# sisl/Crux.jl

Hardware: AMD Instinct MI355X
Metric: env-steps/sec + grad-steps/sec, PPO 2048x32 rollout (higher is better)
Workload: dtype f32

## Files before the change

### crux.jl_amd/csrc/env.hip

```cpp
#include "rollout.h"
#include "per_tree.h"

void crux_buffer_ring_advance(crux_buffer* b, int64_t N);
int32_t crux_buffer_per_on_push(crux_buffer* b, const int64_t* d_I, int64_t N);
int32_t crux_buffer_ring_ids_device(crux_buffer* b, int64_t N, int64_t* d_out);
bool crux_per_push_fused(crux_buffer* b, int64_t n, int64_t* d_ids);
bool crux_per_push_plan(crux_buffer* b, int64_t n, int* touch);
void crux_per_push_done(crux_buffer* b, int touch);

template <int IN, int OUT, int ACT, int KIND>
__global__ __launch_bounds__(64) void k_rollout_h64(RolloutArgs a_single, const RolloutArgs* __restrict__ multi) {
  __shared__ __attribute__((aligned(16))) float sh[64];
  const RolloutArgs a = multi ? multi[blockIdx.x / a_single.E] : a_single;
  const int e = multi ? (int)(blockIdx.x % a_single.E) : (int)blockIdx.x, lane = threadIdx.x;
  const NetDesc& nd = a.nd;
  constexpr int SD = KIND == CRUX_ENV_CARTPOLE ? 4 : ((KIND == CRUX_ENV_SYNTH || KIND == CRUX_ENV_SYNTH_DISCRETE) ? IN : 2);
  float w1[IN], w2[64], w3[OUT], b3[OUT];
#pragma unroll
  for (int k = 0; k < IN; ++k) w1[k] = a.p[nd.woff[0] + lane + 64 * k];
#pragma unroll
  for (int k = 0; k < 64; ++k) w2[k] = a.p[nd.woff[1] + lane + 64 * k];
#pragma unroll
  for (int o = 0; o < OUT; ++o) { w3[o] = a.p[nd.woff[2] + o + OUT * lane]; b3[o] = a.p[nd.boff[2] + o]; }
  const float b1 = a.p[nd.boff[0] + lane], b2 = a.p[nd.boff[1] + lane];
  double st[ENV_MAXSD]; float x[IN], nx[ENV_MAXOBS];
#pragma unroll
  for (int i = 0; i < SD; ++i) st[i] = a.state[(size_t)e * SD + i];
  int64_t ep_len = a.ep_len[e], n_resets = a.n_resets[e], steps_taken = a.steps_taken[e]; double sum_r = 0.0; int64_t nee = 0;
#pragma unroll
  for (int k = 0; k < IN; ++k) x[k] = a.svec[(size_t)e * IN + k];
  for (int64_t t = 0; t < a.T; ++t) {
    const int64_t j = (a.base + (int64_t)e * a.T + t) % a.C;
    if (lane == 0) {
#pragma unroll
      for (int k = 0; k < IN; ++k) a.S[(size_t)j * IN + k] = x[k];
    }
    float z[OUT];
    h64_forward<IN, OUT, ACT>(w1, w2, w3, b3, b1, b2, x, sh, lane, z);
    rollout_tail(a, z, IN, OUT, OUT, KIND, e, t, j, lane == 0, st, ep_len, n_resets, steps_taken, sum_r, nee, nx, lane);
#pragma unroll
    for (int k = 0; k < IN; ++k) x[k] = nx[k];
  }
  if (lane == 0) {
#pragma unroll
    for (int i = 0; i < SD; ++i) a.state[(size_t)e * SD + i] = st[i];
    a.ep_len[e] = ep_len; a.n_resets[e] = n_resets; a.steps_taken[e] = steps_taken;
    a.acc[2 * e] = sum_r; a.acc[2 * e + 1] = (double)nee;
#pragma unroll
    for (int k = 0; k < IN; ++k) a.svec[(size_t)e * IN + k] = x[k];
  }
}

__global__ __launch_bounds__(64) void k_rollout(RolloutArgs a) {
  __shared__ float hbuf[2][1024];
  __shared__ float sh_misc[ENV_MAXOBS + 8];
  rollout_generic_wave(a, blockIdx.x, threadIdx.x, hbuf, sh_misc);
}
__global__ __launch_bounds__(256) void k_rollout_wide(RolloutArgs a) {
  __shared__ float hbuf[2][1024];
  __shared__ float sh_misc[ENV_MAXOBS + 8];
  rollout_generic_wave<256>(a, blockIdx.x, threadIdx.x, hbuf, sh_misc);
}
__global__ __launch_bounds__(64) void k_rollout_sigma(RolloutArgs a) {
  __shared__ float hbuf[2][1024];
  __shared__ float sh_misc[ENV_MAXOBS + 8];
  rollout_generic_wave<64, true>(a, blockIdx.x, threadIdx.x, hbuf, sh_misc);
}
__global__ __launch_bounds__(256) void k_rollout_wide_sigma(RolloutArgs a) {
  __shared__ float hbuf[2][1024];
  __shared__ float sh_misc[ENV_MAXOBS + 8];
  rollout_generic_wave<256, true>(a, blockIdx.x, threadIdx.x, hbuf, sh_misc);
}

__device__ __forceinline__ void env_lds_barrier() { asm volatile("s_waitcnt lgkmcnt(0)\n\ts_barrier" ::: "memory"); }
__device__ __forceinline__ float env_readlane(const float v, const int l) { return __builtin_bit_cast(float, __builtin_amdgcn_readlane(__builtin_bit_cast(int, v), l)); }
template <int L0>
__device__ __forceinline__ void env_rl_fma8(float& acc, const float hreg, const float w0, const float w1, const float w2, const float w3, const float w4, const float w5,
                                            const float w6, const float w7) {
  int t0, t1;
  asm volatile("v_readlane_b32 %[t0], %[h], %[l0]\n\tv_readlane_b32 %[t1], %[h], %[l1]\n\t"
               "v_fmac_f32_e32 %[acc], %[t0], %[w0]\n\tv_readlane_b32 %[t0], %[h], %[l2]\n\t"
               "v_fmac_f32_e32 %[acc], %[t1], %[w1]\n\tv_readlane_b32 %[t1], %[h], %[l3]\n\t"
               "v_fmac_f32_e32 %[acc], %[t0], %[w2]\n\tv_readlane_b32 %[t0], %[h], %[l4]\n\t"
// ... 159 lines not shown
__global__ void k_env_init(int kind, int E, int od, int sd, uint64_t seed, const float* mu, const float* sigma, double* state, int64_t* ep_len,
                           int64_t* n_resets, float* svec, int fresh) {
  const int e = blockIdx.x * blockDim.x + threadIdx.x;
  if (e >= E) return;
  const int64_t nr = fresh ? 0 : n_resets[e];
  if (env_is_synth(kind)) {
    for (int i = 0; i < sd; ++i) { const crux_u32x4 x = crux_philox(seed, 16 * (uint64_t)nr + (uint64_t)(i >> 1), (uint32_t)e, CRUX_RNG_RESET);
      const double ui = (i & 1) ? crux_u32x2_to_f64(x.v[2], x.v[3]) : crux_u32x2_to_f64(x.v[0], x.v[1]); const double xi = __dadd_rn(-0.05, __dmul_rn(0.1, ui));
      state[(size_t)e * sd + i] = xi; svec[(size_t)e * od + i] = __fdiv_rn(__fsub_rn((float)xi, mu[i]), sigma[i]); }
    n_resets[e] = nr + 1; ep_len[e] = 0; return;
  }
  double st[4]; float o[4];
  st[0] = st[1] = st[2] = st[3] = 0.0; o[0] = o[1] = o[2] = o[3] = 0.f;
  env_draw_initial(kind, seed, (uint64_t)nr, (uint32_t)e, st);
#pragma unroll
  for (int i = 0; i < 4; ++i) if (i < sd) state[(size_t)e * sd + i] = st[i];
  n_resets[e] = nr + 1; ep_len[e] = 0;
  env_obs(kind, st, o);
#pragma unroll
  for (int q = 0; q < 4; ++q) if (q < od) svec[(size_t)e * od + q] = __fdiv_rn(__fsub_rn(o[q], mu[q]), sigma[q]);
}

__global__ void k_env_step(int kind, int64_t n, const double* state, const void* action, const double* uniforms, double* next_state, float* obs, float* r, uint8_t* done) {
  const int64_t j = (int64_t)blockIdx.x * blockDim.x + threadIdx.x;
  if (j >= n) return;
  if (kind == CRUX_ENV_GRIDWORLD) {
    const uint8_t* a = (const uint8_t*)action + 4 * j; int act = 0; for (int q = 0; q < 4; ++q) if (a[q]) act = q;
    double s[2] = {state[2 * j], state[2 * j + 1]}, sn[2]; float rr; uint8_t dd;
    gridworld_step(s, act, uniforms ? uniforms[j] : 0.0, sn, &rr, &dd);
    next_state[2 * j] = sn[0]; next_state[2 * j + 1] = sn[1]; obs[2 * j] = (float)sn[0]; obs[2 * j + 1] = (float)sn[1]; r[j] = rr; done[j] = dd; return;
  }
  if (kind == CRUX_ENV_CARTPOLE) {
    const uint8_t* a = (const uint8_t*)action + 2 * j; double s[4], sn[4]; for (int i = 0; i < 4; ++i) s[i] = state[4 * j + i];
    float rr; uint8_t dd; cartpole_step(s, a[1] ? 1 : 0, sn, &rr, &dd);
    for (int i = 0; i < 4; ++i) { next_state[4 * j + i] = sn[i]; obs[4 * j + i] = (float)sn[i]; } r[j] = rr; done[j] = dd;
  } else {
    double s[2] = {state[2 * j], state[2 * j + 1]}, sn[2]; float rr; uint8_t dd; float o[3];
    pendulum_step(s, ((const float*)action)[j], sn, &rr, &dd); env_obs(kind, sn, o);
    next_state[2 * j] = sn[0]; next_state[2 * j + 1] = sn[1]; obs[3 * j] = o[0]; obs[3 * j + 1] = o[1]; obs[3 * j + 2] = o[2]; r[j] = rr; done[j] = dd;
  }
}

static void env_dims(int kind, int so, int sa, int* obs, int* act, int* sd) {
  switch (kind) {
    case CRUX_ENV_CARTPOLE: *obs = 4; *act = 2; *sd = 4; break;
    case CRUX_ENV_PENDULUM: *obs = 3; *act = 1; *sd = 2; break;
    case CRUX_ENV_GRIDWORLD: *obs = 2; *act = 4; *sd = 2; break;
    case CRUX_ENV_SYNTH: case CRUX_ENV_SYNTH_DISCRETE: *obs = so; *act = sa; *sd = so; break;
    default: *obs = so; *act = sa; *sd = 1; break;
  }
}

static bool launch_rollout_h64(const NetDesc& pn, int kind, dim3 grid, hipStream_t stream, const RolloutArgs& a, const RolloutArgs* d_multi) {
#define RO_CASE(I, O, A_, K) if (pn.dims[0] == I && pn.dims[3] == O && pn.acts[0] == A_ && kind == K) { hipLaunchKernelGGL((k_rollout_h64<I, O, A_, K>), grid, dim3(64), 0, stream, a, d_multi); return true; }
  H64_SHAPES(RO_CASE)
#undef RO_CASE
  return false;
}

extern "C" {

int32_t crux_env_create(crux_ctx* ctx, int32_t kind, int32_t n_envs, int32_t max_steps, float gamma, const float* obs_mu, const float* obs_sigma,
                        uint64_t seed, int32_t synth_obs_dim, int32_t synth_act_dim, crux_env** out) {
  if (!ctx || !out) return CRUX_EINVAL;
  if (kind < CRUX_ENV_CARTPOLE || kind > CRUX_ENV_SYNTH_DISCRETE) return crux_fail(ctx, CRUX_EUNSUP, "env kind %d has no device dynamics", kind);
  if ((kind == CRUX_ENV_SYNTH || kind == CRUX_ENV_SYNTH_DISCRETE) && (synth_obs_dim < 1 || synth_obs_dim > ENV_MAXOBS || synth_act_dim < 1 || synth_act_dim > ENV_MAXOBS))
    return crux_fail(ctx, CRUX_EINVAL, "synthetic env: obs/act dims (%d, %d) must be in 1..%d", synth_obs_dim, synth_act_dim, ENV_MAXOBS);
  if (n_envs < 1 || max_steps < 1) return crux_fail(ctx, CRUX_EINVAL, "env_create: n_envs=%d max_steps=%d", n_envs, max_steps);
  crux_env* e = new crux_env(); e->ctx = ctx; e->kind = kind; e->n_envs = n_envs; e->max_steps = max_steps; e->gamma = gamma; e->seed = seed;
  env_dims(kind, synth_obs_dim, synth_act_dim, &e->obs_dim, &e->act_dim, &e->state_dim);
  const int od = e->obs_dim;
  if (hipMalloc(&e->mu, 4 * od) != hipSuccess || hipMalloc(&e->sigma, 4 * od) != hipSuccess || hipMalloc(&e->state, 8 * (size_t)n_envs * e->state_dim) != hipSuccess ||
      hipMalloc(&e->ep_len, 8 * (size_t)n_envs) != hipSuccess || hipMalloc(&e->n_resets, 8 * (size_t)n_envs) != hipSuccess ||
      hipMalloc(&e->steps_taken, 8 * (size_t)n_envs) != hipSuccess || hipMalloc(&e->svec, 4 * (size_t)n_envs * od) != hipSuccess ||
      hipMalloc(&e->acc, 16 * (size_t)n_envs) != hipSuccess) { crux_env_destroy(e); return crux_fail(ctx, CRUX_ENOMEM, "env_create: hipMalloc"); }
  std::vector<float> mu(od, 0.f), sg(od, 1.f);
  if (obs_mu) for (int i = 0; i < od; ++i) mu[i] = obs_mu[i];
  if (obs_sigma) for (int i = 0; i < od; ++i) sg[i] = obs_sigma[i];
  HIPCHK(ctx, hipMemcpyAsync(e->mu, mu.data(), 4 * od, hipMemcpyHostToDevice, ctx->stream));
  HIPCHK(ctx, hipMemcpyAsync(e->sigma, sg.data(), 4 * od, hipMemcpyHostToDevice, ctx->stream));
  HIPCHK(ctx, hipMemsetAsync(e->steps_taken, 0, 8 * (size_t)n_envs, ctx->stream));
  HIPCHK(ctx, hipMemsetAsync(e->acc, 0, 16 * (size_t)n_envs, ctx->stream));
  hipLaunchKernelGGL(k_env_init, dim3((n_envs + 63) / 64), dim3(64), 0, ctx->stream, kind, n_envs, od, e->state_dim, seed, e->mu, e->sigma, e->state, e->ep_len, e->n_resets, e->svec, 1);
  HIPCHK(ctx, hipStreamSynchronize(ctx->stream));
  *out = e; return crux_launch_check(ctx, "k_env_init");
}

int32_t crux_env_destroy(crux_env* e) {
  if (!e) return CRUX_OK;
  crux_sync_before_free(e->ctx);
  (void)hipFree(e->mu); (void)hipFree(e->sigma); (void)hipFree(e->state); (void)hipFree(e->ep_len); (void)hipFree(e->n_resets);
  (void)hipFree(e->steps_taken); (void)hipFree(e->svec); (void)hipFree(e->acc);
  delete e; return CRUX_OK;
}
int32_t crux_env_obs_dim(const crux_env* e) { return e ? e->obs_dim : -1; }
int32_t crux_env_act_dim(const crux_env* e) { return e ? e->act_dim : -1; }
int32_t crux_env_state_dim(const crux_env* e) { return e ? e->state_dim : -1; }

int32_t crux_env_reset(crux_env* e) {
  if (!e) return CRUX_EINVAL;
  hipLaunchKernelGGL(k_env_init, dim3((e->n_envs + 63) / 64), dim3(64), 0, e->ctx->stream, e->kind, e->n_envs, e->obs_dim, e->state_dim, e->seed, e->mu, e->sigma,
                     e->state, e->ep_len, e->n_resets, e->svec, 0);
  return crux_launch_check(e->ctx, "k_env_init");
}

int32_t crux_env_get_state(crux_env* e, double* state, int64_t* ep_len, int64_t* n_resets) {
  if (!e) return CRUX_EINVAL;
// ... 188 lines not shown
```

### crux.jl_amd/csrc/rollout.h

```cpp
#pragma once
#include "common.h"
#define ENV_MAXSD 32
#define ENV_MAXOBS 32
#define PI_D 3.14159265358979323846

__device__ __forceinline__ void cartpole_step(const double* s, int action, double* sn, float* r, uint8_t* done) {
  const double gravity = 9.8, masscart = 1.0, masspole = 0.1, total_mass = masspole + masscart, length = 0.5,
               polemass_length = masspole * length, force_mag = 10.0, tau = 0.02;
  double x = s[0], x_dot = s[1], theta = s[2], theta_dot = s[3];
  const double force = action == 1 ? force_mag : -force_mag;
  const double costheta = cos(theta), sintheta = sin(theta);
  const double temp = __ddiv_rn(__dadd_rn(force, __dmul_rn(__dmul_rn(polemass_length, __dmul_rn(theta_dot, theta_dot)), sintheta)), total_mass);
  const double den = __dmul_rn(length, __dsub_rn(4.0 / 3.0, __ddiv_rn(__dmul_rn(masspole, __dmul_rn(costheta, costheta)), total_mass)));
  const double thetaacc = __ddiv_rn(__dsub_rn(__dmul_rn(gravity, sintheta), __dmul_rn(costheta, temp)), den);
  const double xacc = __dsub_rn(temp, __ddiv_rn(__dmul_rn(__dmul_rn(polemass_length, thetaacc), costheta), total_mass));
  x = __dadd_rn(x, __dmul_rn(tau, x_dot)); x_dot = __dadd_rn(x_dot, __dmul_rn(tau, xacc));
  theta = __dadd_rn(theta, __dmul_rn(tau, theta_dot)); theta_dot = __dadd_rn(theta_dot, __dmul_rn(tau, thetaacc));
  sn[0] = x; sn[1] = x_dot; sn[2] = theta; sn[3] = theta_dot;
  const double xth = 2.4, thth = 12.0 * 2.0 * PI_D / 360.0;
  *done = (x < -xth || x > xth || theta < -thth || theta > thth) ? 1 : 0;
  *r = 1.0f;
}
__device__ __forceinline__ double angle_normalize(double x) { double t = fmod(x + PI_D, 2.0 * PI_D); if (t < 0) t += 2.0 * PI_D; return t - PI_D; }
__device__ __forceinline__ void pendulum_step(const double* s, float a, double* sn, float* r, uint8_t* done) {
// ... 190 lines not shown
                                             const int64_t t, const int64_t j, const bool writer, double* st, int64_t& ep_len, int64_t& n_resets,
                                             int64_t& steps_taken, double& sum_r, int64_t& nee, float* next_obs, const int par_lane = -1,
                                             const float* mu_cached = nullptr, const float* sigma_cached = nullptr) {
  const float* mu = mu_cached ? mu_cached : a.mu; const float* sg = sigma_cached ? sigma_cached : a.sigma;
  const int sd = kind == CRUX_ENV_CARTPOLE ? 4 : (env_is_synth(kind) ? od : 2);
      const uint64_t gi = a.cfg.i0 + (uint64_t)t * (uint64_t)a.E + (uint64_t)e;
      const uint64_t ctr = (uint64_t)steps_taken;
      float logprob; int ai; float aout[ENV_MAXOBS];
      if constexpr (SIGMA) rollout_head_sigma(a, z, ad, e, ctr, aout, ai, logprob); else
      rollout_head(a, z, ad, nout, e, gi, ctr, aout, ai, logprob);
      double sn[ENV_MAXSD]; float r; uint8_t done; float o[ENV_MAXOBS], spv[ENV_MAXOBS];
      if (kind == CRUX_ENV_CARTPOLE) cartpole_step(st, ai, sn, &r, &done);
      else if (kind == CRUX_ENV_PENDULUM) pendulum_step(st, aout[0], sn, &r, &done);
      else if (env_is_synth(kind)) synth_step(od, ad, kind == CRUX_ENV_SYNTH_DISCRETE, st, ai, aout, sn, &r, &done, par_lane);
      else { const crux_u32x4 xd = crux_philox(a.seed, ctr, (uint32_t)e, CRUX_RNG_ENVDYN); gridworld_step(st, ai, crux_u32x2_to_f64(xd.v[0], xd.v[1]), sn, &r, &done); }
      env_obs(kind, sn, o, od);
      for (int q = 0; q < od; ++q) spv[q] = __fdiv_rn(__fsub_rn(o[q], mu[q]), sg[q]);
      if (writer) {
        if (a.act_kind == CRUX_ACTION_DISCRETE) { uint8_t* A = (uint8_t*)a.A + (size_t)j * ad; for (int q = 0; q < ad; ++q) A[q] = aout[q] != 0.f; }
        else { float* A = (float*)a.A + (size_t)j * ad; for (int q = 0; q < ad; ++q) A[q] = aout[q]; }
        for (int q = 0; q < od; ++q) a.SP[(size_t)j * od + q] = spv[q];
        a.R[j] = r; a.D[j] = done;
        if (a.LP) a.LP[j] = logprob;
        if (a.TT) a.TT[j] = ep_len + 1;
        if (a.II) a.II[j] = (int64_t)gi + 1;
        if (a.W) a.W[j] = 1.0f;
        if (a.RET) a.RET[j] = 0.f;
        if (a.ADV) a.ADV[j] = 0.f;
        if (a.COST) a.COST[j] = env_cost(kind, od, sn);
        if (a.CADV) a.CADV[j] = 0.f;
        if (a.CRET) a.CRET[j] = 0.f;
      }
      sum_r += (double)r; steps_taken += 1;
      ep_len += 1;
      uint8_t ee = 0;
      if (done || ep_len >= a.max_steps) {
        ee = 1; ++nee;
        env_draw_initial(kind, a.seed, (uint64_t)n_resets, (uint32_t)e, st, sd); n_resets += 1; ep_len = 0;
        env_obs(kind, st, o, od);
        for (int q = 0; q < od; ++q) next_obs[q] = __fdiv_rn(__fsub_rn(o[q], mu[q]), sg[q]);
      } else {
        for (int i = 0; i < sd; ++i) st[i] = sn[i];
        for (int q = 0; q < od; ++q) next_obs[q] = spv[q];
      }
      if (a.cfg.reset_at_end && t == a.T - 1 && ep_len > 0) {
        ee = 1; ++nee;
        env_draw_initial(kind, a.seed, (uint64_t)n_resets, (uint32_t)e, st, sd); n_resets += 1; ep_len = 0;
        env_obs(kind, st, o, od);
        for (int q = 0; q < od; ++q) next_obs[q] = __fdiv_rn(__fsub_rn(o[q], mu[q]), sg[q]);
      }
      if (writer) a.EE[j] = ee;
}

template <int CTRL> __device__ __forceinline__ float env_dpp(float v) {
  return __builtin_bit_cast(float, __builtin_amdgcn_update_dpp(0, __builtin_bit_cast(int, v), CTRL, 0xf, 0xf, true));
}
__device__ __forceinline__ float env_wave_sum_uniform(float v) {
  v += env_dpp<0x128>(v); v += env_dpp<0x124>(v); v += env_dpp<0x122>(v); v += env_dpp<0x121>(v);
  float a0 = v, b0 = v;
  asm volatile("s_nop 1\n\tv_permlane16_swap_b32 %0, %1\n\ts_nop 1" : "+v"(a0), "+v"(b0));
  a0 = a0 + b0; b0 = a0;
  asm volatile("s_nop 1\n\tv_permlane32_swap_b32 %0, %1\n\ts_nop 1" : "+v"(a0), "+v"(b0));
  return __builtin_bit_cast(float, __builtin_amdgcn_readfirstlane(__builtin_bit_cast(int, a0 + b0)));
}
template <int IN, int OUT, int ACT>
__device__ __forceinline__ void h64_forward(const float (&w1)[IN], const float (&w2)[64], const float (&w3)[OUT], const float (&b3)[OUT], const float b1, const float b2,
                                            const float (&x)[IN], float* sh, const int lane, float (&z)[OUT]) {
    float acc = 0.f;
#pragma unroll
    for (int k = 0; k < IN; ++k) acc = fmaf(w1[k], x[k], acc);
    sh[lane] = crux_act(ACT, acc + b1);
    __builtin_amdgcn_fence(__ATOMIC_ACQ_REL, "wavefront"); __builtin_amdgcn_wave_barrier();
    acc = 0.f;
#pragma unroll
    for (int k4 = 0; k4 < 16; ++k4) { const float4 hv = *(const float4*)&sh[4 * k4];
      acc = fmaf(w2[4 * k4], hv.x, acc); acc = fmaf(w2[4 * k4 + 1], hv.y, acc); acc = fmaf(w2[4 * k4 + 2], hv.z, acc); acc = fmaf(w2[4 * k4 + 3], hv.w, acc); }
    __builtin_amdgcn_fence(__ATOMIC_ACQ_REL, "wavefront"); __builtin_amdgcn_wave_barrier();
    const float h2 = crux_act(ACT, acc + b2);
#pragma unroll
    for (int o = 0; o < OUT; ++o) z[o] = env_wave_sum_uniform(w3[o] * h2) + b3[o];
}
#define RO_WAVE_SYNC() do { __builtin_amdgcn_fence(__ATOMIC_ACQ_REL, "wavefront"); __builtin_amdgcn_wave_barrier(); } while (0)
template <int NT>
__device__ __forceinline__ int rollout_generic_forward(const RolloutArgs& a, const int lane, float (*hbuf)[1024]) {
    const NetDesc& nd = a.nd;
    int cur = 0;
    for (int l = 0; l < nd.L; ++l) {
      const int in = nd.dims[l], out = nd.dims[l + 1], act = nd.acts[l];
      const float* Wl = a.p + nd.woff[l]; const float* bl = a.p + nd.boff[l];
      for (int o = lane; o < out; o += NT) {
        float accv = 0.f; int k = 0;
        if (NT > 64) {
          for (; k + 32 <= in; k += 32) {
            float wv[32];
#pragma unroll
            for (int u = 0; u < 32; ++u) wv[u] = Wl[o + out * (k + u)];
#pragma unroll
            for (int u = 0; u < 32; ++u) accv = fmaf(wv[u], hbuf[cur][k + u], accv); } }
        for (; k + 8 <= in; k += 8) {
          float wv[8];
#pragma unroll
          for (int u = 0; u < 8; ++u) wv[u] = Wl[o + out * (k + u)];
#pragma unroll
          for (int u = 0; u < 8; ++u) accv = fmaf(wv[u], hbuf[cur][k + u], accv); }
        for (; k < in; ++k) accv = fmaf(Wl[o + out * k], hbuf[cur][k], accv);
        hbuf[cur ^ 1][o] = crux_act(act, accv + bl[o]);
// ... 69 lines not shown
```

### crux.jl_amd/csrc/switches.h

```cpp
#pragma once
#include <cstdlib>
struct CruxSwitches {
  bool no_fused_epoch, no_chained_epochs, exec_no_kernarg, force_generic, quiet, verbose, sync_chains, mfma_timing, small_solve_generic, small_solve_timing;
  bool sac_tile_ops, per_fused_gather, pack_rows, spec_pair, dense_pair, mfma_x2;
  int dense_fused;
  int fs;
  bool push_fused;
  bool host_zerocopy;
};
inline CruxSwitches crux_switches_read() {
  auto set = [](const char* k) { return getenv(k) != nullptr; };
  auto not0 = [](const char* k) { const char* e = getenv(k); return !(e && e[0] == '0'); };
  auto num = [](const char* k, int d) { const char* e = getenv(k); return e ? atoi(e) : d; };
  CruxSwitches s{};
  s.no_fused_epoch = set("CRUX_NO_FUSED_EPOCH"); s.no_chained_epochs = set("CRUX_NO_CHAINED_EPOCHS"); s.exec_no_kernarg = set("CRUX_EXEC_NO_KERNARG");
  s.force_generic = set("CRUX_FORCE_GENERIC"); s.quiet = set("CRUX_QUIET"); s.verbose = set("CRUX_VERBOSE"); s.sync_chains = set("CRUX_SYNC_CHAINS");
  s.mfma_timing = set("CRUX_MFMA_TIMING"); s.small_solve_generic = set("CRUX_SMALL_SOLVE_GENERIC"); s.small_solve_timing = set("CRUX_SMALL_SOLVE_TIMING");
  s.sac_tile_ops = not0("CRUX_SAC_TILE_OPS"); s.per_fused_gather = not0("CRUX_PER_FUSED_GATHER"); s.pack_rows = not0("CRUX_PACK_ROWS"); s.spec_pair = not0("CRUX_SPEC_PAIR");
  s.dense_pair = not0("CRUX_DENSE_PAIR"); s.mfma_x2 = not0("CRUX_MFMA_X2"); s.push_fused = not0("CRUX_PUSH_FUSED"); s.host_zerocopy = not0("CRUX_HOST_ZEROCOPY");
  { const char* e = getenv("CRUX_DENSE_FUSED"); s.dense_fused = !e ? 1 : e[0] == '0' ? 0 : e[0] == '2' ? 2 : 1; }
  s.fs = num("CRUX_FS", 1);
  return s;
}
const CruxSwitches& crux_sw();
```

### crux.jl_amd/csrc/train.hip

```cpp
#include "learner_route.h"
#include <thread>
#include "exec.h"
#include "ops_small.h"

int32_t crux_buffer_apply_order(crux_buffer* b, const int32_t* d_order, int64_t n);
int32_t crux_buffer_apply_order_multi(int32_t n, crux_buffer* const* bufs, const int32_t* const* d_orders);
int32_t crux_launch_fs2(crux_ctx* c, const TrainArgs& a, const LearnerShape* row, hipStream_t stream);
int32_t crux_launch_x2(crux_ctx* c, const TrainArgs& a, const LearnerShape* row, hipStream_t stream);
int32_t crux_launch_x2_multi(crux_ctx* c, std::vector<TrainArgs>& as, const LearnerShape* row, hipStream_t stream);
int32_t crux_launch_one8(crux_ctx* c, const TrainArgs& a, const LearnerShape* row, hipStream_t stream);
int32_t crux_launch_one8_multi(crux_ctx* c, std::vector<TrainArgs>& as, const LearnerShape* row, hipStream_t stream);
int32_t crux_train_dense_run(crux_ctx* c, TrainArgs& a, hipStream_t strm = nullptr, int which = 0, const crux_fisher* reg = nullptr);
extern "C" int crux_x2_placement_ok(crux_ctx* c);
static RouteEnv route_env(crux_ctx* c) { return RouteEnv{crux_sw(), c->learner_cus, crux_grouped(c), c->peer_every, [c]() { return crux_x2_placement_ok(c) != 0; }}; }

#include "train_generic.h"
__global__ __launch_bounds__(256) void k_train_generic(TrainArgs a) {
  extern __shared__ __attribute__((aligned(16))) float sm[];
  __shared__ double red[4];
  train_generic_run(a, sm, red);
}

extern "C" const char* crux_peer_why_text(int why);
extern "C" int32_t crux_peer_abort_reason(crux_ctx* c, int32_t* out2);
static int32_t learner_stopped(crux_ctx* c, int why, const char* sfx) {
  if (why >= 16 || why == 3) { int32_t ab[2] = {0, 0}; if (crux_grouped(c)) (void)crux_peer_abort_reason(c, ab); const int who = ab[0] ? ab[0] : ab[1];
    return crux_fail(c, CRUX_EHIP, "learner kernel stopped%s, replica group: %s%s%s. The group is ended: detach and attach again", sfx, crux_peer_why_text(why >= 16 ? why - 16 : 0),
                     (why - 16 == 3 && who) ? " -- " : "", (why - 16 == 3 && who) ? crux_peer_why_text(who) : ""); }
  return crux_fail(c, CRUX_EHIP, "learner kernel stopped%s: %s", sfx, why == 2 ? "its workgroups were placed on different XCDs (concurrent dispatches interleaved them)" :
                   why == 4 ? "a workgroup never arrived at the abort-latch consensus of a speculatively started learner" : "one of its workgroups never arrived at the exchange (or the replica group's abort word was raised)");
}
static int32_t learner_status(crux_ctx* c, const int32_t* st, const int32_t* st2 = nullptr, const char* who = "learner kernel", const char* sfx = "") {
  const int32_t e1 = st[0], e2 = st2 ? st2[0] : 0;
  if (e1 == CRUX_ENAN || e2 == CRUX_ENAN) return crux_fail(c, CRUX_ENAN, "NaN detected! (grad norm is NaN, src/training.jl:20)%s", sfx);
  if (e1 == CRUX_EHIP || e2 == CRUX_EHIP) return learner_stopped(c, e1 == CRUX_EHIP ? st[4] : st2[4], sfx);
  if (!e1 && !e2) return CRUX_OK;
  if (!st2) return crux_fail(c, e1, "%s reported status %d%s", who, e1, sfx);
  return crux_fail(c, e1 ? e1 : e2, "%s reported status %d/%d%s", who, e1, e2, sfx);
}
static void reduce_infos(int batches, int epochs, const float* ei, float* info_out, float* epoch_infos) {
  if (info_out) {
    for (int q = 0; q < CRUX_INFO_N; ++q) { double s = 0; for (int e = 0; e < epochs; ++e) s += (double)ei[(size_t)e * CRUX_INFO_N + q]; info_out[q] = epochs ? (float)(s / (double)epochs) : 0.f; }
    info_out[CRUX_INFO_BATCHES_TRAINED] = (float)batches; info_out[CRUX_INFO_EPOCHS_RUN] = (float)epochs;
  }
  if (epoch_infos) memcpy(epoch_infos, ei, sizeof(float) * CRUX_INFO_N * (size_t)epochs);
}
static int32_t fill_args(TrainArgs& a, crux_mlp* net, crux_buffer* buf, const crux_train_cfg* cfg, int internal_loss) {
  crux_ctx* c = net->ctx;
  if (!net->has_adam) return crux_fail(c, CRUX_EINVAL, "train!: crux_adam_init was not called for this network");
  if (net->nd.dims[0] != buf->obs_dim) return crux_fail(c, CRUX_EINVAL, "train!: network input %d != obs dim %d", net->nd.dims[0], buf->obs_dim);
  memset(&a, 0, sizeof a);
  a.px_timeout = net->ctx->peer_timeout_ticks;
  train_args_net(a, net);
// ... 1 lines not shown
  a.LP = has_col(buf, CRUX_COL_LOGPROB) ? (const float*)buf->col[CRUX_COL_LOGPROB] : nullptr;
  a.ADV = has_col(buf, CRUX_COL_ADVANTAGE) ? (const float*)buf->col[CRUX_COL_ADVANTAGE] : nullptr;
  a.RET = has_col(buf, CRUX_COL_RETURN) ? (const float*)buf->col[CRUX_COL_RETURN] : nullptr;
  a.od = buf->obs_dim; a.ad = buf->act_dim; a.act_kind = buf->act_kind;
  a.loss = internal_loss; a.head = cfg->head; a.bs = cfg->batch_size; a.epochs = cfg->epochs; a.max_batches = cfg->max_batches;
  a.eps_clip = cfg->eps_clip; a.lambda_p = cfg->lambda_p; a.lambda_e = cfg->lambda_e; a.target_kl = cfg->target_kl;
  a.shuffle_seed = cfg->shuffle_seed; a.shuffle_counter = cfg->shuffle_counter;
  a.len = buf->elements; a.order_a = buf->order_a; a.order_b = buf->order_b; a.apply = 1; a.squash = net->squash; a.host_net = net;
  const int nout = net->nd.dims[net->nd.L];
  if (internal_loss == CRUX_LOSS_LOGPDF_BC) {
    if (!buf->aux_ones) {
      if (hipMalloc(&buf->aux_ones, 4 * (size_t)buf->capacity) != hipSuccess || hipMalloc(&buf->aux_zeros, 4 * (size_t)buf->capacity) != hipSuccess) return crux_fail(c, CRUX_ENOMEM, "logpdf_bc_loss: constant columns");
      std::vector<float> one((size_t)buf->capacity, 1.f);
      HIPCHK(c, hipMemcpyAsync(buf->aux_ones, one.data(), 4 * one.size(), hipMemcpyHostToDevice, c->stream)); HIPCHK(c, hipMemsetAsync(buf->aux_zeros, 0, 4 * (size_t)buf->capacity, c->stream));
      HIPCHK(c, hipStreamSynchronize(c->stream));
    }
    a.ADV = buf->aux_ones; a.LP = buf->aux_zeros; a.lambda_p = 1.f; a.loss = internal_loss = CRUX_LOSS_A2C;
  }
  if (internal_loss == CRUX_LOSS_REINFORCE) {
    if (!a.RET || !a.LP) return crux_fail(c, CRUX_EINVAL, "reinforce_loss: buffer needs :return and :logprob columns");
    a.ADV = a.RET; a.lambda_p = 1.f; a.lambda_e = 0.f; a.loss = internal_loss = CRUX_LOSS_A2C;
  }
  if (CRUX_IS_PG(internal_loss)) {
    if (!a.LP || !a.ADV) return crux_fail(c, CRUX_EINVAL, "ppo_loss: buffer needs :logprob and :advantage columns");
    if (net->sigma_head && cfg->head == CRUX_HEAD_GAUSSIAN) {
      if (nout != 2 * buf->act_dim || net->nd.n_extra != 0 || buf->act_kind != CRUX_ACTION_CONTINUOUS)
        return crux_fail(c, CRUX_EINVAL, "ppo_loss: a two-headed gaussian head needs 2 x %d output rows (mu, then logSigma), no extras and a Float32 action column (got %d rows, %d extras)", buf->act_dim, nout, net->nd.n_extra); }
    else if (cfg->head == CRUX_HEAD_CATEGORICAL) { if (nout != buf->act_dim || buf->act_kind != CRUX_ACTION_DISCRETE || nout > 32) return crux_fail(c, CRUX_EINVAL, "ppo_loss: categorical head needs %d logits over a one-hot action column", buf->act_dim); }
    else if (cfg->head == CRUX_HEAD_GAUSSIAN) { if (nout != buf->act_dim || buf->act_kind != CRUX_ACTION_CONTINUOUS || net->nd.n_extra != buf->act_dim) return crux_fail(c, CRUX_EINVAL, "ppo_loss: gaussian head needs %d means + %d logSigma extras over a Float32 action column", buf->act_dim, buf->act_dim); }
    else return crux_fail(c, CRUX_EINVAL, "ppo_loss: head %d unsupported", cfg->head);
  } else if (internal_loss == CRUX_LOSS_VALUE_MSE) {
    if (cfg->target_col > 0) {
      const int k = cfg->target_col;
      if (!has_col(buf, k) || col_rows(buf, k) != 1 || col_elem(buf, k) != 4) return crux_fail(c, CRUX_EINVAL, "critic mse: target column %d is not a Float32 row of this buffer", k);
      a.RET = (const float*)buf->col[k];
    }
    if (!a.RET || nout != 1) return crux_fail(c, CRUX_EINVAL, "critic mse: needs a :return column and a scalar-output network");
  } else if (internal_loss == CRUX_LOSS_MSE_ACTION && net->sigma_head) {
    return crux_fail(c, CRUX_EUNSUP, "mse_action_loss on a two-headed Gaussian actor (logSigma network) is not implemented: its learners are ppo_loss, a2c_loss, reinforce_loss and logpdf_bc_loss");
  } else if (internal_loss == CRUX_LOSS_MSE_ACTION && net->squash > 0.f) {
    return crux_fail(c, CRUX_EUNSUP, "mse_action_loss through a SquashedGaussianPolicy (ascale*tanh(mu)) is not implemented");
  } else if (internal_loss == CRUX_LOSS_MSE_ACTION) {
    if (buf->act_kind != CRUX_ACTION_CONTINUOUS || nout != buf->act_dim) return crux_fail(c, CRUX_EINVAL, "mse_action_loss: needs a continuous action column of %d rows", nout);
  }
  if (cfg->batch_size < 1) return crux_fail(c, CRUX_EINVAL, "train!: batch_size %d", cfg->batch_size);
  return CRUX_OK;
}

__global__ void k_compose_order(const int32_t* __restrict__ prev, int32_t* __restrict__ out, crux_perm pp, const int64_t* __restrict__ perm_explicit, int64_t len) {
  const int64_t j = (int64_t)blockIdx.x * blockDim.x + threadIdx.x; if (j >= len) return;
  const int64_t src = perm_explicit ? perm_explicit[j] : (int64_t)crux_perm_at(&pp, (uint32_t)j);
  out[j] = prev ? prev[src] : (int32_t)src;
}
static int32_t ensure_ord(crux_ctx* c, crux_buffer* buf, int slot, size_t need) {
  if (buf->ord_all_cap[slot] < need) {
    if (buf->ord_all[slot]) { if (!c->peer_same_device) HIPCHK(c, hipDeviceSynchronize()); (void)hipFree(buf->ord_all[slot]); buf->ord_all[slot] = nullptr; buf->ord_all_cap[slot] = 0; }
    if (hipMalloc(&buf->ord_all[slot], 4 * need) != hipSuccess) return crux_fail(c, CRUX_ENOMEM, "batch_train!: %zu bytes for the epoch orders", 4 * need);
    buf->ord_all_cap[slot] = need;
  }
  return CRUX_OK;
}
static int32_t build_orders(crux_ctx* c, crux_buffer* buf, int slot, const int32_t* start, uint64_t seed, uint64_t counter, const int64_t* d_perms, int n_epochs, hipStream_t st, int32_t** out) {
  const int64_t len = buf->elements; const size_t need = (size_t)n_epochs * (size_t)len;
  { const int32_t rc0 = ensure_ord(c, buf, slot, need); if (rc0) return rc0; }
  const int32_t* prev = start;
  for (int e = 0; e < n_epochs; ++e) {
    int32_t* o = buf->ord_all[slot] + (size_t)e * (size_t)len;
    crux_perm pp = crux_perm_make(seed, counter + (uint64_t)e, 0, (uint32_t)len);
    hipLaunchKernelGGL(k_compose_order, dim3((unsigned)((len + 255) / 256)), dim3(256), 0, st, prev, o, pp, d_perms ? d_perms + (size_t)e * (size_t)len : (const int64_t*)nullptr, len);
    prev = o;
  }
  *out = buf->ord_all[slot];
  return crux_launch_check(c, "k_compose_order");
}

__global__ void k_pack_rows(const float* __restrict__ S, const void* __restrict__ A, int act_kind, const float* __restrict__ LP, const float* __restrict__ ADV, const float* __restrict__ RET,
                            int od, int ad, int64_t n, int stride, float* __restrict__ out) {
  const int64_t t = (int64_t)blockIdx.x * blockDim.x + threadIdx.x; const int64_t row = t / stride; const int e = (int)(t - row * stride);
  if (row >= n) return;
  const int na = act_kind == CRUX_ACTION_DISCRETE ? 1 : ad;
  float v = 0.f;
  if (e < od) v = S[row * od + e];
  else if (e < od + na) { if (act_kind == CRUX_ACTION_DISCRETE) { int ai = 0; const uint8_t* a = (const uint8_t*)A + row * ad; for (int k = 0; k < ad; ++k) ai = a[k] ? k : ai; v = (float)ai; }
                          else v = ((const float*)A)[row * ad + (e - od)]; }
  else if (e == od + na) v = LP ? LP[row] : 0.f;
  else if (e == od + na + 1) v = ADV ? ADV[row] : 0.f;
  else if (e == od + na + 2) v = RET ? RET[row] : 0.f;
  out[t] = v;
}
static int32_t ensure_pack(crux_ctx* c, crux_buffer* buf, hipStream_t st, TrainArgs& a, TrainArgs* k) {
  if (!crux_sw().pack_rows) return CRUX_OK;
  const int od = buf->obs_dim, ad = buf->act_dim, na = buf->act_kind == CRUX_ACTION_DISCRETE ? 1 : ad; const int need = od + na + 3;
  if (need > 64 || a.lag || a.ids) return CRUX_OK;
  const float* ret = has_col(buf, CRUX_COL_RETURN) ? (const float*)buf->col[CRUX_COL_RETURN] : nullptr;
  if ((a.RET && a.RET != ret) || (k && k->RET && k->RET != ret)) return CRUX_OK;
  int stride = 8; while (stride < need) stride *= 2;
  const size_t fl = (size_t)buf->capacity * (size_t)stride;
  if (buf->pack_floats < fl) { if (buf->pack) { crux_sync_before_free(c); (void)hipFree(buf->pack); buf->pack = nullptr; buf->pack_floats = 0; }
    if (hipMalloc(&buf->pack, 4 * fl) != hipSuccess) { buf->pack = nullptr; return CRUX_OK; }
    buf->pack_floats = fl; }
  const int64_t n = buf->elements, tot = n * stride;
  hipLaunchKernelGGL(k_pack_rows, dim3((unsigned)((tot + 255) / 256)), dim3(256), 0, st, (const float*)buf->col[CRUX_COL_S], (const void*)buf->col[CRUX_COL_A], buf->act_kind,
                     has_col(buf, CRUX_COL_LOGPROB) ? (const float*)buf->col[CRUX_COL_LOGPROB] : (const float*)nullptr, has_col(buf, CRUX_COL_ADVANTAGE) ? (const float*)buf->col[CRUX_COL_ADVANTAGE] : (const float*)nullptr, ret,
                     od, ad, n, stride, buf->pack);
  TrainArgs* both[2] = {&a, k};
  for (int q = 0; q < 2; ++q) { TrainArgs* t = both[q]; if (!t) continue;
    const bool plain = (t->LP == nullptr || t->LP == (const float*)buf->col[CRUX_COL_LOGPROB]) && (t->ADV == nullptr || (has_col(buf, CRUX_COL_ADVANTAGE) && t->ADV == (const float*)buf->col[CRUX_COL_ADVANTAGE]));
    if (!plain && t->loss != CRUX_LOSS_VALUE_MSE) continue;
    t->PACK = buf->pack; t->pack_stride = stride; t->pack_act = od; t->pack_lp = od + na; }
  return crux_launch_check(c, "k_pack_rows");
}
static int32_t launch_train(crux_ctx* c, TrainArgs& a, int prof_slot, hipStream_t stream = nullptr, const crux_fisher* reg = nullptr) {
  if (!stream) stream = c->stream;
  const RoutePlan plan = learner_route(route_env(c), a, reg != nullptr, a.ord_all != nullptr);
  if (plan.code) return crux_fail(c, plan.code, "%s", plan.msg);
  a.need_px = plan.need_px; a.px_every = plan.px_every; a.px_timeout = c->peer_timeout_ticks;
  const bool prof = stream == c->stream;
  if (prof) crux_prof_begin(c, prof_slot);
// ... 591 lines not shown
```

Before: 322,300.

## Add lean specialized rollout tail with batched RNG draws and blocked epoch-order composition

```diff
diff --git a/crux.jl_amd/csrc/env.hip b/crux.jl_amd/csrc/env.hip
--- a/crux.jl_amd/csrc/env.hip
+++ b/crux.jl_amd/csrc/env.hip
@@ -9,7 +9,7 @@
 void crux_per_push_done(crux_buffer* b, int touch);
 
 template <int IN, int OUT, int ACT, int KIND>
-__global__ __launch_bounds__(64) void k_rollout_h64(RolloutArgs a_single, const RolloutArgs* __restrict__ multi) {
+__global__ __launch_bounds__(64) void k_rollout_h64(RolloutArgs a_single, const RolloutArgs* __restrict__ multi, const int lean_sw) {
   __shared__ __attribute__((aligned(16))) float sh[64];
   const RolloutArgs a = multi ? multi[blockIdx.x / a_single.E] : a_single;
   const int e = multi ? (int)(blockIdx.x % a_single.E) : (int)blockIdx.x, lane = threadIdx.x;
@@ -29,6 +29,32 @@
   int64_t ep_len = a.ep_len[e], n_resets = a.n_resets[e], steps_taken = a.steps_taken[e]; double sum_r = 0.0; int64_t nee = 0;
 #pragma unroll
   for (int k = 0; k < IN; ++k) x[k] = a.svec[(size_t)e * IN + k];
+  constexpr bool LG = KIND == CRUX_ENV_PENDULUM || KIND == CRUX_ENV_SYNTH, LC = KIND == CRUX_ENV_CARTPOLE;
+  const bool lean = lean_sw && a.cfg.explore == 1 && ((LG && a.cfg.head == CRUX_HEAD_GAUSSIAN) || (LC && a.cfg.head == CRUX_HEAD_CATEGORICAL && a.cfg.eps_steps <= 0));
+  if constexpr (LG || LC) if (lean) {
+    constexpr int PER = LG ? 64 / OUT : 64;
+    float mu[IN], sg[IN], ls[OUT], sgm[OUT];
+#pragma unroll
+    for (int k = 0; k < IN; ++k) { mu[k] = a.mu[k]; sg[k] = a.sigma[k]; }
+#pragma unroll
+    for (int q = 0; q < OUT; ++q) { ls[q] = LG ? a.p[nd.xoff + q] : 0.f; sgm[q] = LG ? expf(a.squash > 0.f ? sq_clampls(ls[q]) : ls[q]) : 0.f; }
+    int slot = PER; uint32_t drawv = 0;
+    int64_t j = (a.base + (int64_t)e * a.T) % a.C; uint64_t gi = a.cfg.i0 + (uint64_t)e;
+    for (int64_t t = 0; t < a.T; ++t) {
+      if (slot == PER) { drawv = lean_draw_block<OUT, LG>(a.seed, (uint64_t)steps_taken, e, lane); slot = 0; }
+      if (lane == 0) {
+#pragma unroll
+        for (int k = 0; k < IN; ++k) a.S[(size_t)j * IN + k] = x[k];
+      }
+      float z[OUT];
+      h64_forward<IN, OUT, ACT>(w1, w2, w3, b3, b1, b2, x, sh, lane, z);
+      rollout_tail_lean<IN, OUT, KIND, LG>(a, z, e, t == a.T - 1, j, gi, lane == 0, drawv, slot, mu, sg, ls, sgm, st, ep_len, n_resets, steps_taken, sum_r, nee, nx, lane);
+#pragma unroll
+      for (int k = 0; k < IN; ++k) x[k] = nx[k];
+      ++slot; ++j; if (j == a.C) j = 0; gi += (uint64_t)a.E;
+    }
+  }
+  if (!lean)
   for (int64_t t = 0; t < a.T; ++t) {
     const int64_t j = (a.base + (int64_t)e * a.T + t) % a.C;
     if (lane == 0) {
@@ -294,7 +320,7 @@
 }
 
 static bool launch_rollout_h64(const NetDesc& pn, int kind, dim3 grid, hipStream_t stream, const RolloutArgs& a, const RolloutArgs* d_multi) {
-#define RO_CASE(I, O, A_, K) if (pn.dims[0] == I && pn.dims[3] == O && pn.acts[0] == A_ && kind == K) { hipLaunchKernelGGL((k_rollout_h64<I, O, A_, K>), grid, dim3(64), 0, stream, a, d_multi); return true; }
+#define RO_CASE(I, O, A_, K) if (pn.dims[0] == I && pn.dims[3] == O && pn.acts[0] == A_ && kind == K) { hipLaunchKernelGGL((k_rollout_h64<I, O, A_, K>), grid, dim3(64), 0, stream, a, d_multi, crux_sw().rollout_lean ? 1 : 0); return true; }
   H64_SHAPES(RO_CASE)
 #undef RO_CASE
   return false;
diff --git a/crux.jl_amd/csrc/order_block.h b/crux.jl_amd/csrc/order_block.h
--- /dev/null
+++ b/crux.jl_amd/csrc/order_block.h
@@ -0,0 +1,8 @@
+#pragma once
+#include "../../include/crux_rng.h"
+#define CRUX_ORDER_BLOCK_MAX 16
+CRUX_HD uint32_t order_walk(const crux_perm* pp, int k, uint32_t j) {
+  for (int i = k - 1; i >= 0; --i) j = crux_perm_at(&pp[i], j);
+  return j;
+}
+template <int K> struct crux_perm_block { crux_perm p[K]; };
diff --git a/crux.jl_amd/csrc/rollout.h b/crux.jl_amd/csrc/rollout.h
--- a/crux.jl_amd/csrc/rollout.h
+++ b/crux.jl_amd/csrc/rollout.h
@@ -266,6 +266,99 @@
       if (writer) a.EE[j] = ee;
 }
 
+template <int AD, bool GAUSS>
+__device__ __forceinline__ uint32_t lean_draw_block(const uint64_t seed, const uint64_t ctr0, const int e, const int lane) {
+  if constexpr (GAUSS) {
+    uint32_t v = 0;
+    if (lane < AD * (64 / AD)) { const int q = lane % AD;
+      v = __builtin_bit_cast(uint32_t, randn_f32(seed, (ctr0 + (uint64_t)(lane / AD)) * (uint64_t)((AD + 1) / 2) + (uint64_t)(q / 2), (uint32_t)e, q & 1)); }
+    return v;
+  } else return crux_philox(seed, ctr0 + (uint64_t)lane, (uint32_t)e, CRUX_RNG_ACTION).v[0];
+}
+template <int IN, int OUT, int KIND, bool GAUSS>
+__device__ __forceinline__ void rollout_tail_lean(const RolloutArgs& a, const float (&z)[OUT], const int e, const bool last, const int64_t j, const uint64_t gi, const bool writer,
+                                                  const uint32_t drawv, const int slot, const float (&mu)[IN], const float (&sg)[IN], const float (&ls)[OUT], const float (&sgm)[OUT],
+                                                  double* st, int64_t& ep_len, int64_t& n_resets, int64_t& steps_taken, double& sum_r, int64_t& nee, float* next_obs, const int lane) {
+  constexpr int SD = KIND == CRUX_ENV_CARTPOLE ? 4 : ((KIND == CRUX_ENV_SYNTH || KIND == CRUX_ENV_SYNTH_DISCRETE) ? IN : 2);
+  float logprob; int ai = 0; float aout[OUT];
+  if constexpr (!GAUSS) {
+    float pr[OUT], zq[OUT];
+    const float ldiv = a.cfg.logit_div > 0.f ? a.cfg.logit_div : 1.f;
+#pragma unroll
+    for (int q = 0; q < OUT; ++q) zq[q] = __fdiv_rn(z[q], ldiv);
+    float mx = zq[0];
+#pragma unroll
+    for (int q = 1; q < OUT; ++q) mx = zq[q] > mx ? zq[q] : mx;
+    float sum = 0.f;
+#pragma unroll
+    for (int q = 0; q < OUT; ++q) { pr[q] = expf(zq[q] - mx); sum = __fadd_rn(sum, pr[q]); }
+#pragma unroll
+    for (int q = 0; q < OUT; ++q) pr[q] = __fdiv_rn(pr[q], sum);
+    const float draw = crux_u32_to_f32((uint32_t)__builtin_amdgcn_readlane((int)drawv, slot));
+    float cp = pr[0], pai = pr[0]; bool go = true;
+#pragma unroll
+    for (int q = 1; q < OUT; ++q) { go = go && cp <= draw; if (go) { ai = q; pai = pr[q]; cp = __fadd_rn(cp, pr[q]); } }
+    logprob = logf(pai);
+#pragma unroll
+    for (int q = 0; q < OUT; ++q) aout[q] = (q == ai) ? 1.f : 0.f;
+  } else {
+    float lp = 0.f;
+#pragma unroll
+    for (int q = 0; q < OUT; ++q) {
+      const float m = z[q], sgq = sgm[q];
+      const float epsn = __builtin_bit_cast(float, __builtin_amdgcn_readlane((int)drawv, slot * OUT + q));
+      const float u = __fadd_rn(__fmul_rn(epsn, sgq), m); const float s2 = __fmul_rn(sgq, sgq); const float dd = __fsub_rn(u, m);
+      const float t0 = __fsub_rn(__fsub_rn(__fdiv_rn(-__fmul_rn(dd, dd), __fmul_rn(2.f, s2)), 0.9189385332046727f), ls[q]);
+      if (a.squash > 0.f) { aout[q] = __fmul_rn(a.squash, tanhf(u)); lp = __fadd_rn(lp, __fsub_rn(t0, sq_corr(u))); }
+      else { aout[q] = u; lp = __fadd_rn(lp, t0); }
+    }
+    logprob = lp;
+  }
+  double sn[SD]; float r; uint8_t done; float o[IN], spv[IN];
+  if constexpr (KIND == CRUX_ENV_CARTPOLE) cartpole_step(st, ai, sn, &r, &done);
+  else if constexpr (KIND == CRUX_ENV_PENDULUM) pendulum_step(st, aout[0], sn, &r, &done);
+  else synth_step(IN, OUT, KIND == CRUX_ENV_SYNTH_DISCRETE, st, ai, aout, sn, &r, &done, lane);
+  env_obs(KIND, sn, o, IN);
+#pragma unroll
+  for (int q = 0; q < IN; ++q) spv[q] = __fdiv_rn(__fsub_rn(o[q], mu[q]), sg[q]);
+  if (writer) {
+    if (a.act_kind == CRUX_ACTION_DISCRETE) { uint8_t* A = (uint8_t*)a.A + (size_t)j * OUT;
+#pragma unroll
+      for (int q = 0; q < OUT; ++q) A[q] = aout[q] != 0.f; }
+    else { float* A = (float*)a.A + (size_t)j * OUT;
+#pragma unroll
+      for (int q = 0; q < OUT; ++q) A[q] = aout[q]; }
+#pragma unroll
+    for (int q = 0; q < IN; ++q) a.SP[(size_t)j * IN + q] = spv[q];
+    a.R[j] = r; a.D[j] = done;
+    if (a.LP) a.LP[j] = logprob;
+    if (a.TT) a.TT[j] = ep_len + 1;
+    if (a.II) a.II[j] = (int64_t)gi + 1;
+    if (a.W) a.W[j] = 1.0f;
+    if (a.RET) a.RET[j] = 0.f;
+    if (a.ADV) a.ADV[j] = 0.f;
+    if (a.COST) a.COST[j] = env_cost(KIND, IN, sn);
+    if (a.CADV) a.CADV[j] = 0.f;
+    if (a.CRET) a.CRET[j] = 0.f;
+  }
+  sum_r += (double)r; steps_taken += 1;
+  ep_len += 1;
+  const bool ee = done || ep_len >= a.max_steps || (a.cfg.reset_at_end && last);
+  if (ee) {
+    ++nee;
+    env_draw_initial(KIND, a.seed, (uint64_t)n_resets, (uint32_t)e, st, SD); n_resets += 1; ep_len = 0;
+    env_obs(KIND, st, o, IN);
+#pragma unroll
+    for (int q = 0; q < IN; ++q) next_obs[q] = __fdiv_rn(__fsub_rn(o[q], mu[q]), sg[q]);
+  } else {
+#pragma unroll
+    for (int i = 0; i < SD; ++i) st[i] = sn[i];
+#pragma unroll
+    for (int q = 0; q < IN; ++q) next_obs[q] = spv[q];
+  }
+  if (writer) a.EE[j] = ee ? 1 : 0;
+}
+
 template <int CTRL> __device__ __forceinline__ float env_dpp(float v) {
   return __builtin_bit_cast(float, __builtin_amdgcn_update_dpp(0, __builtin_bit_cast(int, v), CTRL, 0xf, 0xf, true));
 }
diff --git a/crux.jl_amd/csrc/switches.h b/crux.jl_amd/csrc/switches.h
--- a/crux.jl_amd/csrc/switches.h
+++ b/crux.jl_amd/csrc/switches.h
@@ -6,6 +6,8 @@
   int dense_fused;
   int fs;
   bool push_fused;
+  bool rollout_lean;
+  int order_block;
   bool host_zerocopy;
 };
 inline CruxSwitches crux_switches_read() {
@@ -20,6 +22,7 @@
   s.dense_pair = not0("CRUX_DENSE_PAIR"); s.mfma_x2 = not0("CRUX_MFMA_X2"); s.push_fused = not0("CRUX_PUSH_FUSED"); s.host_zerocopy = not0("CRUX_HOST_ZEROCOPY");
   { const char* e = getenv("CRUX_DENSE_FUSED"); s.dense_fused = !e ? 1 : e[0] == '0' ? 0 : e[0] == '2' ? 2 : 1; }
   s.fs = num("CRUX_FS", 1);
+  s.rollout_lean = not0("CRUX_ROLLOUT_LEAN"); s.order_block = num("CRUX_ORDER_BLOCK", 8);
   return s;
 }
 const CruxSwitches& crux_sw();
diff --git a/crux.jl_amd/csrc/train.hip b/crux.jl_amd/csrc/train.hip
--- a/crux.jl_amd/csrc/train.hip
+++ b/crux.jl_amd/csrc/train.hip
@@ -1,4 +1,5 @@
 #include "learner_route.h"
+#include "order_block.h"
 #include <thread>
 #include "exec.h"
 #include "ops_small.h"
@@ -106,6 +107,23 @@
   const int64_t src = perm_explicit ? perm_explicit[j] : (int64_t)crux_perm_at(&pp, (uint32_t)j);
   out[j] = prev ? prev[src] : (int32_t)src;
 }
+template <int K>
+__global__ void k_compose_order_block(const int32_t* __restrict__ prev, int32_t* __restrict__ out, const crux_perm_block<K> pb, const int nk, const int64_t len) {
+  const int64_t j = (int64_t)blockIdx.x * blockDim.x + threadIdx.x; if (j >= len) return;
+#pragma unroll
+  for (int k = 1; k <= K; ++k) if (k <= nk) {
+    const uint32_t s = order_walk(pb.p, k, (uint32_t)j);
+    out[(size_t)(k - 1) * (size_t)len + (size_t)j] = prev ? prev[s] : (int32_t)s;
+  }
+}
+template <int K>
+static int compose_block(const int32_t* prev, int32_t* out, uint64_t seed, uint64_t counter, int left, int64_t len, hipStream_t st) {
+  const int nk = left < K ? left : K;
+  crux_perm_block<K> pb;
+  for (int i = 0; i < K; ++i) pb.p[i] = crux_perm_make(seed, counter + (uint64_t)i, 0, (uint32_t)len);
+  hipLaunchKernelGGL(k_compose_order_block<K>, dim3((unsigned)((len + 255) / 256)), dim3(256), 0, st, prev, out, pb, nk, len);
+  return nk;
+}
 static int32_t ensure_ord(crux_ctx* c, crux_buffer* buf, int slot, size_t need) {
   if (buf->ord_all_cap[slot] < need) {
     if (buf->ord_all[slot]) { if (!c->peer_same_device) HIPCHK(c, hipDeviceSynchronize()); (void)hipFree(buf->ord_all[slot]); buf->ord_all[slot] = nullptr; buf->ord_all_cap[slot] = 0; }
@@ -118,6 +136,17 @@
   const int64_t len = buf->elements; const size_t need = (size_t)n_epochs * (size_t)len;
   { const int32_t rc0 = ensure_ord(c, buf, slot, need); if (rc0) return rc0; }
   const int32_t* prev = start;
+  const int K = d_perms ? 1 : crux_sw().order_block;
+  if (K > 1) {
+    for (int e0 = 0; e0 < n_epochs; ) {
+      int32_t* o = buf->ord_all[slot] + (size_t)e0 * (size_t)len;
+      const int done = K >= 16 ? compose_block<16>(prev, o, seed, counter + (uint64_t)e0, n_epochs - e0, len, st) : K >= 8 ? compose_block<8>(prev, o, seed, counter + (uint64_t)e0, n_epochs - e0, len, st)
+                                                                                                                    : compose_block<4>(prev, o, seed, counter + (uint64_t)e0, n_epochs - e0, len, st);
+      e0 += done; prev = o + (size_t)(done - 1) * (size_t)len;
+    }
+    *out = buf->ord_all[slot];
+    return crux_launch_check(c, "k_compose_order_block");
+  }
   for (int e = 0; e < n_epochs; ++e) {
     int32_t* o = buf->ord_all[slot] + (size_t)e * (size_t)len;
     crux_perm pp = crux_perm_make(seed, counter + (uint64_t)e, 0, (uint32_t)len);
```

Result: no change. 324,500 (median of 6 runs) (+0.7%).
